# rezasalatin/PINN_depthEstimation

Hardware: AMD Instinct MI355X
Metric: collocation-point residuals/sec (fwd+PDE-grad+Adam) (higher is better)
Workload: dtype f32; 1 GPU; BASELINE configs[1]: 3->8x64 tanh->4 MLP, Navier_Stokes residual, 1048576 synthetic (t,x,y) points per GPU, full-batch Adam step; points_per_gpu=1048576, global_points=1048576, params=29636, parallelism=dp1, engine=0, allreduce_bytes=0

## Files before the change

pinn_depthestimation_amd/csrc/fused_kernel.h:

```cpp
#pragma once
#include <string.h>
#include <type_traits>
#include "common.h"
#include "residuals.h"

namespace pinn {

typedef float f4 __attribute__((ext_vector_type(4)));

constexpr int FUSED_WAVES = 4;
constexpr int FUSED_W16_WAVES = 3;
constexpr int FUSED_FLUSH_ROWS = 4;
constexpr int FUSED_THREADS = FUSED_WAVES * 64;
constexpr int TB_FLOATS = 256;
constexpr int TB_PER_WAVE = 8;
constexpr int MAX_SUMS = 12;
constexpr int MSE_SUM0 = 4;

struct FusedParams {
  int d_in, d_out, L, act;
  int dir_col[PINN_MAX_DIRS];
  int64_t N, n_tiles;
  const float* X;
  const float* Wp;
  const float* WTp;
  const float* Bp;
  float* scratch;
  int64_t scratch_per_wave;
  float* Y; float* dY;
  int loss_kind;
  int residual_id;
  int out_col[PINN_MAX_ROLES];
  int q_of[PINN_MAX_DIRS];
  float thr, anchor; int xcol;
  const float* scale;
  int n_cols;
  int mse_col[PINN_MAX_ROLES];
  const float* T;
  int64_t n_split;
  const float* mse_scale;
  float* wg_sums;
  float* wg_grads;
  int acc_lds;
  int PW, PB;
  int lds_acc_floats;
  int batch_T;
  int io1;
  uint32_t drop_seed, drop_thresh;
  float drop_scale, drop_keep;
  const float* gY;
  const float* gdY;
};

inline void set_residual_roles(FusedParams& P, const Net& n, const pinn_residual_spec& spec) {
  P.residual_id = spec.residual_id;
  for (int j = 0; j < PINN_MAX_ROLES; ++j) P.out_col[j] = spec.out_col[j];
  for (int d = 0; d < PINN_MAX_DIRS; ++d) P.q_of[d] = 1 + spec.dir_of[d];
  P.thr = spec.param[0]; P.anchor = spec.param[1];
  P.xcol = n.dir_col[spec.dir_of[0]];
}
inline void set_loss(FusedParams& P, const Net& n, const LossReq& rq) {
  P.n_split = rq.n_split;
  P.loss_kind = rq.kind == 0 ? 1 : (rq.kind == 1 ? 2 : 3);
  if (P.loss_kind & 1) { P.scale = rq.scale; set_residual_roles(P, n, rq.spec); }
  else for (int j = 0; j < PINN_MAX_ROLES; ++j) P.out_col[j] = -1;
  if (P.loss_kind & 2) {
    P.n_cols = rq.n_cols; P.T = rq.T; P.mse_scale = rq.mse_scale;
    for (int j = 0; j < PINN_MAX_ROLES; ++j) P.mse_col[j] = j < rq.n_cols ? rq.out_col[j] : -1;
  }
}

__device__ __forceinline__ f4 mfma4(float a, float b, f4 c) {
  return __builtin_amdgcn_mfma_f32_16x16x4f32(a, b, c, 0, 0, 0);
}

template <int WP> __device__ __forceinline__ int w_off_p(int l) { return l == 0 ? 0 : WP * 16 + (l - 1) * WP * WP; }
template <int WP> __device__ __forceinline__ int b_off_p(int l) { return l * WP; }

template <int NT_IN, int NT_OUT>
__device__ __forceinline__ void load_w(const float* __restrict__ Wl, f4 (&w)[NT_OUT][NT_IN], int m, int kq) {
  constexpr int LDW = 16 * NT_IN;
#pragma unroll
  for (int MT = 0; MT < NT_OUT; ++MT)
#pragma unroll
    for (int kt = 0; kt < NT_IN; ++kt)
      w[MT][kt] = *reinterpret_cast<const f4*>(Wl + (16 * MT + m) * LDW + 16 * kt + 4 * kq);
}

template <int NT_IN, int NT_OUT, int K1, int KR = 4>
__device__ __forceinline__ void gemm_chain(const f4 (&w)[NT_OUT][NT_IN], const f4 (&bin)[K1][NT_IN],
                                           f4 (&acc)[K1][NT_OUT]) {
#pragma unroll
  for (int MT = 0; MT < NT_OUT; ++MT)
#pragma unroll
    for (int kt = 0; kt < NT_IN; ++kt)
#pragma unroll
      for (int r = 0; r < KR; ++r)
#pragma unroll
        for (int c = 0; c < K1; ++c) acc[c][MT] = mfma4(w[MT][kt][r], bin[c][kt][r], acc[c][MT]);
}


template <int NT_IN>
__device__ __forceinline__ void load_wblk(const float* __restrict__ Wl, int MT, f4 (&w)[NT_IN], int m, int kq) {
#pragma unroll
  for (int kt = 0; kt < NT_IN; ++kt)
    w[kt] = *reinterpret_cast<const f4*>(Wl + (16 * MT + m) * (16 * NT_IN) + 16 * kt + 4 * kq);
}

struct NoMid { __device__ __forceinline__ void operator()() const {} };
template <int NT_IN, int NT_OUT, int K1, class Mid = NoMid>
__device__ __forceinline__ void gemm_stream(const float* __restrict__ Wl, const float* __restrict__ Wnext,
                                            f4 (&wa)[NT_IN], const f4 (&bin)[K1][NT_IN], f4 (&acc)[K1][NT_OUT],
                                            int m, int kq, const Mid& mid = Mid()) {
  constexpr int MID_BLOCK = NT_OUT >= 3 ? 1 : 0;
#pragma unroll
  for (int MT = 0; MT < NT_OUT; ++MT) {
    f4 wb[NT_IN];
    if (MT + 1 < NT_OUT) load_wblk<NT_IN>(Wl, MT + 1, wb, m, kq);
    else load_wblk<NT_IN>(Wnext, 0, wb, m, kq);
    if (MT == MID_BLOCK) mid();
#pragma unroll
    for (int kt = 0; kt < NT_IN; ++kt)
#pragma unroll
      for (int r = 0; r < 4; ++r)
#pragma unroll
        for (int c = 0; c < K1; ++c) acc[c][MT] = mfma4(wa[kt][r], bin[c][kt][r], acc[c][MT]);
    __builtin_amdgcn_sched_barrier(0);
#pragma unroll
    for (int kt = 0; kt < NT_IN; ++kt) wa[kt] = wb[kt];
  }
}

template <int NT, int K1>
__device__ __forceinline__ void zero_tiles(f4 (&v)[K1][NT]) {
#pragma unroll
  for (int c = 0; c < K1; ++c)
#pragma unroll
    for (int MT = 0; MT < NT; ++MT) v[c][MT] = f4{0.f, 0.f, 0.f, 0.f};
}

template <int NT, int K1>
__device__ __forceinline__ void init_bias(const float* __restrict__ b, f4 (&acc)[K1][NT], int q) {
#pragma unroll
  for (int MT = 0; MT < NT; ++MT) {
    acc[0][MT] = *reinterpret_cast<const f4*>(b + 16 * MT + 4 * q);
#pragma unroll
    for (int c = 1; c < K1; ++c) acc[c][MT] = f4{0.f, 0.f, 0.f, 0.f};
  }
}

template <int ACT, int NT, int K1>
__device__ __forceinline__ void activate(f4 (&acc)[K1][NT]) {
#pragma unroll
  for (int MT = 0; MT < NT; ++MT)
#pragma unroll
    for (int r = 0; r < 4; ++r) {
      const float z = acc[0][MT][r];
      float a, s;
      if constexpr (ACT == PINN_ACT_TANH) { a = tanh_f32(z); s = fmaf(-a, a, 1.f); }
      else { a = z > 0.f ? z : 0.01f * z; s = z > 0.f ? 1.f : 0.01f; }
      acc[0][MT][r] = a;
#pragma unroll
      for (int c = 1; c < K1; ++c) acc[c][MT][r] *= s;
    }
}

template <int ACT, int NT, int K1>
__device__ __forceinline__ void activate_adjoint(f4 (&G)[K1][NT], const f4 (&A)[K1][NT]) {
#pragma unroll
  for (int MT = 0; MT < NT; ++MT)
#pragma unroll
    for (int r = 0; r < 4; ++r) {
      const float a = A[0][MT][r];
      if constexpr (ACT == PINN_ACT_TANH) {
        const float s = fmaf(-a, a, 1.f);
        float cross = 0.f;
#pragma unroll
        for (int c = 1; c < K1; ++c) {
          cross = fmaf(G[c][MT][r], A[c][MT][r], cross);
          G[c][MT][r] *= s;
        }
        G[0][MT][r] = fmaf(-2.f * a, cross, s * G[0][MT][r]);
      } else {
        const float s = a > 0.f ? 1.f : 0.01f;
#pragma unroll
        for (int c = 0; c < K1; ++c) G[c][MT][r] *= s;
      }
    }
}


struct DropLane {
  uint32_t h0, hi, thresh;
  float scale, keep_p;
  __device__ __forceinline__ void init(uint32_t seed, uint32_t thr, float sc, float kp, int64_t point) {
    h0 = dropout_fmix(seed ^ ((uint32_t)point * 0x9E3779B1u));
    hi = (uint32_t)((uint64_t)point >> 32);
    thresh = thr; scale = sc; keep_p = kp;
  }
  __device__ __forceinline__ float mask(int layer, int unit) const {
    const uint32_t x = h0 ^ (((uint32_t)layer * 0x01000193u + (uint32_t)unit) * 0x9E3779B1u + hi);
    return dropout_fmix(x) >= thresh ? scale : 0.f;
  }
};

template <int NT>
__device__ __forceinline__ void load_bias(const float* __restrict__ b, f4 (&bias)[NT], int q) {
#pragma unroll
  for (int MT = 0; MT < NT; ++MT) bias[MT] = *reinterpret_cast<const f4*>(b + 16 * MT + 4 * q);
}
template <int ACT, int NT, int K1, bool DROP = false>
__device__ __forceinline__ void activate_to(const f4 (&acc)[K1][NT], const f4 (&bias)[NT], f4 (&a)[K1][NT],
                                            const DropLane* dl = nullptr, int layer = 0, int q = 0) {
  if constexpr (ACT == PINN_ACT_TANH && !DROP) {
#pragma unroll
    for (int MT = 0; MT < NT; ++MT)
#pragma unroll
      for (int h = 0; h < 4; h += 2) {
        const f2 z = f2{acc[0][MT][h], acc[0][MT][h + 1]} + f2{bias[MT][h], bias[MT][h + 1]};
        const f2 av = tanh_f32x2(z);
        const f2 s = __builtin_elementwise_fma(-av, av, f2{1.f, 1.f});
        a[0][MT][h] = av[0]; a[0][MT][h + 1] = av[1];
#pragma unroll
        for (int c = 1; c < K1; ++c) {
          const f2 t = f2{acc[c][MT][h], acc[c][MT][h + 1]} * s;
          a[c][MT][h] = t[0]; a[c][MT][h + 1] = t[1];
        }
      }
    return;
  }
#pragma unroll
  for (int MT = 0; MT < NT; ++MT)
#pragma unroll
    for (int r = 0; r < 4; ++r) {
      const float z = acc[0][MT][r] + bias[MT][r];
      float av, s;
      if constexpr (ACT == PINN_ACT_TANH) { av = tanh_f32(z); s = fmaf(-av, av, 1.f); }
      else { av = z > 0.f ? z : 0.01f * z; s = z > 0.f ? 1.f : 0.01f; }
      if constexpr (DROP) {
        const float m = dl->mask(layer, 16 * MT + 4 * q + r);
        av *= m; s *= m;
      }
      a[0][MT][r] = av;
#pragma unroll
      for (int c = 1; c < K1; ++c) a[c][MT][r] = acc[c][MT][r] * s;
    }
}
template <int ACT, int NT, int K1, bool DROP = false>
__device__ __forceinline__ void activate_adjoint_to(const f4 (&G)[K1][NT], const f4 (&A)[K1][NT], f4 (&Z)[K1][NT],
                                                    const DropLane* dl = nullptr, int layer = 0, int q = 0) {
#pragma unroll
  for (int MT = 0; MT < NT; ++MT)
#pragma unroll
    for (int r = 0; r < 4; ++r) {
      float a = A[0][MT][r];
      if constexpr (DROP) a *= dl->keep_p;
      if constexpr (ACT == PINN_ACT_TANH) {
        float s = fmaf(-a, a, 1.f);
        if constexpr (DROP) s *= dl->mask(layer, 16 * MT + 4 * q + r);
        float cross = 0.f;
#pragma unroll
        for (int c = 1; c < K1; ++c) {
          cross = fmaf(G[c][MT][r], A[c][MT][r], cross);
          Z[c][MT][r] = G[c][MT][r] * s;
        }
        Z[0][MT][r] = fmaf(-2.f * a, cross, s * G[0][MT][r]);
      } else {
        const float s = a > 0.f ? 1.f : 0.01f;
#pragma unroll
        for (int c = 0; c < K1; ++c) Z[c][MT][r] = G[c][MT][r] * s;
      }
    }
}

template <int NT, int K1>
__device__ __forceinline__ void activate_sin_to(const f4 (&acc)[K1][NT], const f4 (&bias)[NT], f4 (&a)[K1][NT],
                                                const float* __restrict__ W0, const float* __restrict__ xrow, int d_in, int q) {
#pragma unroll
  for (int MT = 0; MT < NT; ++MT)
#pragma unroll
    for (int r = 0; r < 4; ++r) {
      float sn, cs;
      sincos_f64arg(sin_layer_z(W0 + (16 * MT + 4 * q + r) * 16, bias[MT][r], xrow, d_in), sn, cs);
      a[0][MT][r] = sn;
#pragma unroll
      for (int c = 1; c < K1; ++c) a[c][MT][r] = acc[c][MT][r] * cs;
    }
}
template <int NT, int K1, int KRI>
__device__ __forceinline__ void sin_adjoint_to(const float* __restrict__ W0, const float* __restrict__ B0, const f4 (&in)[K1][1],
                                               const f4 (&G)[K1][NT], f4 (&Z)[K1][NT], int p, int q,
                                               const float* __restrict__ xrow, int d_in) {
  f4 w0[NT][1];
  load_w<1, NT>(W0, w0, p, q);
  f4 bias[NT];
  load_bias<NT>(B0, bias, q);
  f4 cz[NT], sz[NT], cross[NT];
#pragma unroll
  for (int MT = 0; MT < NT; ++MT) {
    cross[MT] = f4{0.f, 0.f, 0.f, 0.f};
#pragma unroll
    for (int r = 0; r < 4; ++r) {
      float sn, cs;
      sincos_f64arg(sin_layer_z(W0 + (16 * MT + 4 * q + r) * 16, bias[MT][r], xrow, d_in), sn, cs);
      sz[MT][r] = sn; cz[MT][r] = cs;
    }
  }
#pragma unroll
  for (int c = 1; c < K1; ++c) {
    f4 bv[1][1], zd[1][NT];
    bv[0][0] = in[c][0];
    zero_tiles<NT, 1>(zd);
    gemm_chain<1, NT, 1, KRI>(w0, bv, zd);
#pragma unroll
    for (int MT = 0; MT < NT; ++MT)
#pragma unroll
      for (int r = 0; r < 4; ++r) {
        cross[MT][r] = fmaf(G[c][MT][r], zd[0][MT][r], cross[MT][r]);
        Z[c][MT][r] = G[c][MT][r] * cz[MT][r];
      }
  }
#pragma unroll
  for (int MT = 0; MT < NT; ++MT)
#pragma unroll
    for (int r = 0; r < 4; ++r) Z[0][MT][r] = fmaf(-sz[MT][r], cross[MT][r], cz[MT][r] * G[0][MT][r]);
}

template <int NT, int K1>
__device__ __forceinline__ void spill(float* __restrict__ slot, const f4 (&v)[K1][NT], int lane) {
#pragma unroll
  for (int c = 0; c < K1; ++c)
#pragma unroll
    for (int MT = 0; MT < NT; ++MT) *reinterpret_cast<f4*>(slot + (c * NT + MT) * 256 + lane * 4) = v[c][MT];
}
template <int NT, int K1>
__device__ __forceinline__ void unspill(const float* __restrict__ slot, f4 (&v)[K1][NT], int lane) {
#pragma unroll
  for (int c = 0; c < K1; ++c)
#pragma unroll
    for (int MT = 0; MT < NT; ++MT) v[c][MT] = *reinterpret_cast<const f4*>(slot + (c * NT + MT) * 256 + lane * 4);
}

__device__ __forceinline__ void transpose_write(float* __restrict__ tb, f4 v, int p, int q) {
  *reinterpret_cast<f4*>(tb + p * 16 + 4 * (q ^ (p & 3))) = v;
}
template <bool CONSECUTIVE = false>
__device__ __forceinline__ f4 transpose_read(const float* __restrict__ tb, int p, int q) {
  f4 o;
#pragma unroll
  for (int s = 0; s < 4; ++s) {
    const int pt = CONSECUTIVE ? 4 * q + s : 4 * s + q;
    o[s] = tb[pt * 16 + 4 * ((p >> 2) ^ (pt & 3)) + (p & 3)];
  }
  return o;
}

__device__ __forceinline__ void transpose_write2(float* __restrict__ tb, f4 v, int p, int q) {
  float* d = tb + (4 * q) * 16 + 4 * (((p >> 2) + 2 * q) & 3) + (p & 3);
#pragma unroll
  for (int r = 0; r < 4; ++r) d[r * 16] = v[r];
}
__device__ __forceinline__ f4 transpose_read2(const float* __restrict__ tb, int p, int q) {
  return *reinterpret_cast<const f4*>(tb + p * 16 + 4 * ((q + 2 * (p >> 2)) & 3));
}

__device__ __forceinline__ float add_xor16(float t) {
  const auto r = __builtin_amdgcn_permlane16_swap(__float_as_uint(t), __float_as_uint(t), false, false);
  return __uint_as_float(r[0]) + __uint_as_float(r[1]);
}
__device__ __forceinline__ float add_xor32(float t) {
  const auto r = __builtin_amdgcn_permlane32_swap(__float_as_uint(t), __float_as_uint(t), false, false);
  return __uint_as_float(r[0]) + __uint_as_float(r[1]);
}

constexpr int MAX_LOCKS = 128;

template <bool LDSACC>
struct GradSink {
  static constexpr bool LDS = LDSACC;
  float* acc;
  int* locks;
  __device__ __forceinline__ void lock(int l, int lane) const {
    if (lane == 0) {
      int expected = 0;
      while (!__hip_atomic_compare_exchange_strong(locks + l, &expected, 1, __ATOMIC_ACQUIRE, __ATOMIC_RELAXED,
                                                   __HIP_MEMORY_SCOPE_WORKGROUP)) {
        expected = 0;
        __builtin_amdgcn_s_sleep(1);
      }
    }
    __builtin_amdgcn_fence(__ATOMIC_ACQUIRE, "workgroup");
    __builtin_amdgcn_wave_barrier();
  }
  __device__ __forceinline__ void unlock(int l, int lane) const {
    __builtin_amdgcn_wave_barrier();
    __builtin_amdgcn_fence(__ATOMIC_RELEASE, "workgroup");
    if (lane == 0) __hip_atomic_store(locks + l, 0, __ATOMIC_RELEASE, __HIP_MEMORY_SCOPE_WORKGROUP);
  }
  __device__ __forceinline__ void add1(int idx, float v) const { acc[idx] += v; }
};

template <int MT_N, int NT_N, int K1, bool UNIT_A = false, class Sink>
__device__ __forceinline__ void weight_grad(const Sink& sink, int layer, int woff, int boff, const f4 (&Z)[K1][MT_N],
                                            const f4 (&A)[K1][NT_N], float* __restrict__ tb, int lane,
                                            const int* __restrict__ dir_col = nullptr) {
  static_assert(!UNIT_A || NT_N == 1, "unit tangents: the layer-0 input block");
  const int p = lane & 15, q = lane >> 4;
  f4 dw[MT_N][NT_N];
  float bs[MT_N], bcur[MT_N];
#pragma unroll
  for (int MT = 0; MT < MT_N; ++MT)
#pragma unroll
    for (int NT = 0; NT < NT_N; ++NT) dw[MT][NT] = f4{0.f, 0.f, 0.f, 0.f};
  f4 early[Sink::LDS ? 1 : MT_N][Sink::LDS ? 1 : NT_N];
  if constexpr (!Sink::LDS) {
    sink.lock(layer, lane);
#pragma unroll
    for (int MT = 0; MT < MT_N; ++MT)
#pragma unroll
      for (int NT = 0; NT < NT_N; ++NT)
        early[MT][NT] = *reinterpret_cast<const f4*>(sink.acc + woff + ((MT * NT_N + NT) * 64 + lane) * 4);
  }
  f4 zt[2][MT_N], at[2][NT_N];
  auto stage = [&](int c, f4 (&z)[MT_N], f4 (&a)[NT_N]) {
#pragma unroll
    for (int MT = 0; MT < MT_N; ++MT) transpose_write2(tb + MT * TB_FLOATS, Z[c][MT], p, q);
    const bool unit = UNIT_A && c > 0;
    if (!unit) {
#pragma unroll
      for (int NT = 0; NT < NT_N; ++NT) transpose_write2(tb + (4 + NT) * TB_FLOATS, A[c][NT], p, q);
    }
#pragma unroll
    for (int MT = 0; MT < MT_N; ++MT) z[MT] = transpose_read2(tb + MT * TB_FLOATS, p, q);
    if (!unit) {
#pragma unroll
      for (int NT = 0; NT < NT_N; ++NT) a[NT] = transpose_read2(tb + (4 + NT) * TB_FLOATS, p, q);
    } else {
      const float e = (p == dir_col[c - 1]) ? 1.f : 0.f;
      a[0] = f4{e, e, e, e};
    }
  };
  stage(0, zt[0], at[0]);
#pragma unroll
  for (int c = 0; c < K1; ++c) {
    __builtin_amdgcn_sched_barrier(0);
    if (c + 1 < K1) stage(c + 1, zt[(c + 1) & 1], at[(c + 1) & 1]);
    __builtin_amdgcn_sched_barrier(0);
    if (c == 0) {
#pragma unroll
      for (int MT = 0; MT < MT_N; ++MT) bs[MT] = (zt[0][MT][0] + zt[0][MT][1]) + (zt[0][MT][2] + zt[0][MT][3]);
    }
#pragma unroll
    for (int s = 0; s < 4; ++s)
#pragma unroll
      for (int MT = 0; MT < MT_N; ++MT)
#pragma unroll
        for (int NT = 0; NT < NT_N; ++NT) dw[MT][NT] = mfma4(zt[c & 1][MT][s], at[c & 1][NT][s], dw[MT][NT]);
  }
#pragma unroll
  for (int MT = 0; MT < MT_N; ++MT) {
    bs[MT] = add_xor32(add_xor16(bs[MT]));
  }
  if constexpr (!Sink::LDS) {
#pragma unroll
    for (int MT = 0; MT < MT_N; ++MT)
#pragma unroll
      for (int NT = 0; NT < NT_N; ++NT)
        *reinterpret_cast<f4*>(sink.acc + woff + ((MT * NT_N + NT) * 64 + lane) * 4) = early[MT][NT] + dw[MT][NT];
  } else {
    sink.lock(layer, lane);
    constexpr int FR = FUSED_FLUSH_ROWS < MT_N ? FUSED_FLUSH_ROWS : MT_N;
#pragma unroll
    for (int M0 = 0; M0 < MT_N; M0 += FR) {
      f4 cur[FR][NT_N];
#pragma unroll
      for (int MT = M0; MT < M0 + FR && MT < MT_N; ++MT)
#pragma unroll
        for (int NT = 0; NT < NT_N; ++NT)
          cur[MT - M0][NT] = *reinterpret_cast<const f4*>(sink.acc + woff + ((MT * NT_N + NT) * 64 + lane) * 4);
      if (M0 == 0) {
#pragma unroll
        for (int MT = 0; MT < MT_N; ++MT) bcur[MT] = sink.acc[boff + 16 * MT + p];
      }
      __builtin_amdgcn_sched_barrier(0);
      __builtin_amdgcn_sched_barrier(0);
#pragma unroll
      for (int MT = M0; MT < M0 + FR && MT < MT_N; ++MT)
#pragma unroll
        for (int NT = 0; NT < NT_N; ++NT)
          *reinterpret_cast<f4*>(sink.acc + woff + ((MT * NT_N + NT) * 64 + lane) * 4) = cur[MT - M0][NT] + dw[MT][NT];
    }
  }
  if (q == 0) {
#pragma unroll
    for (int MT = 0; MT < MT_N; ++MT) {
      if constexpr (Sink::LDS) sink.acc[boff + 16 * MT + p] = bcur[MT] + bs[MT];
      else sink.add1(boff + 16 * MT + p, bs[MT]);
    }
  }
  sink.unlock(layer, lane);
}

__device__ __forceinline__ float pick4(f4 v, int i) {
  return i == 0 ? v[0] : (i == 1 ? v[1] : (i == 2 ? v[2] : v[3]));
}
__device__ __forceinline__ float gather_out(f4 tile, int o, int p) {
  return __shfl(pick4(tile, o & 3), p + 16 * (o >> 2), 64);
}
__device__ __forceinline__ f4 select4(bool take, f4 a, f4 b) { return take ? a : b; }
template <int K1>
__device__ __forceinline__ f4 pick_q(const f4 (&out)[K1][1], int qi) {
  f4 v = out[0][0];
#pragma unroll
  for (int c = 1; c < K1; ++c) v = select4(qi == c, out[c][0], v);
  return v;
}

template <int K1>
struct ScatterMap {
  int role_of[4];
  int cinv[K1];
};

template <int K1, int NC, int NR, bool ACCUM = false>
__device__ __forceinline__ void scatter_adjoint(float* __restrict__ tb, const float (&g)[NC][NR],
                                                const ScatterMap<K1>& sm, f4 (&G)[K1][1], bool valid, int p, int q) {
  if (q == 0) {
#pragma unroll
    for (int c = 0; c < NC; ++c)
#pragma unroll
      for (int r = 0; r < NR; ++r) tb[(c * NR + r) * 16 + p] = g[c][r];
  }
  __builtin_amdgcn_wave_barrier();
#pragma unroll
  for (int ce = 0; ce < K1; ++ce)
#pragma unroll
    for (int r2 = 0; r2 < 4; ++r2) {
      const int ci = sm.cinv[ce], ro = sm.role_of[r2];
      const bool ok = valid && ci >= 0 && ci < NC && ro >= 0;
      const float val = tb[ok ? (ci * NR + ro) * 16 + p : p];
      G[ce][0][r2] = (ACCUM ? G[ce][0][r2] : 0.f) + (ok ? val : 0.f);
    }
  __builtin_amdgcn_wave_barrier();
}

template <class RES, int K1, bool GRAD>
__device__ __forceinline__ void residual_tile(const FusedParams& P, const f4 (&out)[K1][1], f4 (&G)[K1][1],
                                              float (&sums)[MAX_SUMS], const ScatterMap<K1>& sm,
                                              float* __restrict__ tb, bool valid, bool masked, int p, int q,
                                              bool primary = true) {
  constexpr int NR = RES::NR, ND = RES::ND, NT = RES::NT;
  float v[1 + ND][NR], g[1 + ND][NR], sq[NT], sc[NT];
#pragma unroll
  for (int c = 0; c <= ND; ++c) {
    const f4 tile = (c == 0) ? out[0][0] : pick_q<K1>(out, P.q_of[c - 1]);
#pragma unroll
    for (int r = 0; r < NR; ++r) v[c][r] = gather_out(tile, P.out_col[r], p);
  }
#pragma unroll
  for (int t = 0; t < NT; ++t) sc[t] = GRAD ? P.scale[t] : 0.f;
  if constexpr (std::is_same<RES, ResContinuity>::value)
    RES::template eval<GRAD>(v, sc, g, sq, P.residual_id == PINN_RES_CONTINUITY_ONLY, masked, P.anchor);
  else
    RES::template eval<GRAD>(v, sc, g, sq);
  if (valid && q == 0 && primary) {
#pragma unroll
    for (int t = 0; t < NT; ++t) sums[t] += sq[t];
  }
  if constexpr (GRAD) scatter_adjoint<K1, 1 + ND, NR>(tb, g, sm, G, valid, p, q);
}

template <int K1>
__device__ __forceinline__ void build_scatter_maps(const FusedParams& P, int q, ScatterMap<K1>& sm, ScatterMap<K1>& sm_mse) {
#pragma unroll
  for (int r2 = 0; r2 < 4; ++r2) {
    int ro = -1, rm = -1;
    for (int r = PINN_MAX_ROLES - 1; r >= 0; --r) {
      ro = (P.out_col[r] == 4 * q + r2) ? r : ro;
      rm = (r < P.n_cols && P.mse_col[r] == 4 * q + r2) ? r : rm;
    }
    sm.role_of[r2] = ro;
    sm_mse.role_of[r2] = rm;
  }
  sm.cinv[0] = 0; sm_mse.cinv[0] = 0;
#pragma unroll
  for (int ce = 1; ce < K1; ++ce) {
    int ci = -1;
    for (int d = PINN_MAX_DIRS - 1; d >= 0; --d) ci = (P.q_of[d] == ce) ? 1 + d : ci;
    sm.cinv[ce] = ci;
    sm_mse.cinv[ce] = -1;
  }
}

constexpr int EPI_GENERIC = 0, EPI_NS = 1, EPI_PE = 2, EPI_CONT = 3, EPI_ADJ = 4, EPI_FIELD = 5, EPI_PEC = 6, EPI_FIELD_PEC = 7,
              EPI_COEF = 8, EPI_WEIGHTED = 9;
constexpr int COEF_SUM = 3;

template <int K1>
__device__ __forceinline__ void load_adjoint(const FusedParams& P, f4 (&G)[K1][1], int64_t pt, bool valid, int q) {
#pragma unroll
  for (int r = 0; r < 4; ++r) {
    const int o = 4 * q + r;
    const bool ok = valid && o < P.d_out;
    G[0][0][r] = (ok && P.gY != nullptr) ? P.gY[pt * P.d_out + o] : 0.f;
#pragma unroll
    for (int c = 1; c < K1; ++c)
      G[c][0][r] = (ok && P.gdY != nullptr) ? P.gdY[((int64_t)(c - 1) * P.N + pt) * P.d_out + o] : 0.f;
  }
}

template <class RES, int K1>
// ... 307 lines not shown
```

pinn_depthestimation_amd/csrc/fused_tile_body.inc:

```
  constexpr bool IO1 = KRO > 0;
  constexpr int KRI = IO1 ? 1 : 4;
  constexpr int KRL = IO1 ? KRO : 4;
  extern __shared__ __attribute__((aligned(16))) float smem[];
  constexpr int NTH = WP / 16;
  constexpr bool SIN0 = ACT == PINN_ACT_SIN_TANH;
  constexpr int ACT_H = SIN0 ? PINN_ACT_TANH : ACT;
  const int lane = threadIdx.x & 63, wave = threadIdx.x >> 6;
  const int p = lane & 15, q = lane >> 4;
  float* lacc = smem;
  int* locks = reinterpret_cast<int*>(smem + P.lds_acc_floats);
  float* tb = smem + P.lds_acc_floats + MAX_LOCKS + wave * (TB_PER_WAVE * TB_FLOATS);
  float* lsum = smem + P.lds_acc_floats + MAX_LOCKS + FUSED_WAVES * TB_PER_WAVE * TB_FLOATS;
  const int PP = P.PW + P.PB;
  GradSink<LDSACC> sink;
  sink.acc = LDSACC ? lacc : P.wg_grads + (int64_t)blockIdx.x * PP;
  sink.locks = locks;
  if (GRAD) {
    if (LDSACC) {
      for (int i = threadIdx.x; i < PP; i += FUSED_THREADS) lacc[i] = 0.f;
    }
    if (threadIdx.x < MAX_LOCKS) locks[threadIdx.x] = 0;
    __syncthreads();
  }
  float sums[MAX_SUMS];
#pragma unroll
  for (int j = 0; j < MAX_SUMS; ++j) sums[j] = 0.f;

  ScatterMap<K1> sm, sm_mse;
  build_scatter_maps<K1>(P, q, sm, sm_mse);
  const int nw = gridDim.x * FUSED_WAVES;
  const int gw = EPI == EPI_ADJ ? wave * (int)gridDim.x + (int)blockIdx.x : (int)blockIdx.x * FUSED_WAVES + wave;
  float* __restrict__ scr = P.scratch + (int64_t)gw * P.scratch_per_wave;
  const float* __restrict__ Wp_ = P.Wp;
  const float* __restrict__ WTp_ = P.WTp;
  const float* __restrict__ Bp_ = P.Bp;
  constexpr int SLOT = K1 * NTH * 256;
  const int L = P.L;

#ifdef PINN_DIAG
  unsigned long long diag[12] = {0, 0, 0, 0, 0, 0, 0, 0, 0, 0, 0, 0}, tprev = __builtin_amdgcn_s_memtime();
#endif
  auto load_x = [&](int64_t t, f4& x) {
    int64_t pc = t * 16 + p;
    pc = pc < P.N ? pc : P.N - 1;
#pragma unroll
    for (int r = 0; r < 4; ++r) {
      const int f = IO1 ? (r == 0 ? q : 16) : 4 * q + r;
      x[r] = (f < P.d_in) ? P.X[pc * P.d_in + f] : 0.f;
    }
  };
  f4 xnext;
  load_x(gw < P.n_tiles ? gw : 0, xnext);
  for (int64_t tile = gw; tile < P.n_tiles; tile += nw) {
    PINN_STAMP(11);
    const int64_t pt = tile * 16 + p;
    const bool valid = pt < P.N;
    const int64_t ptc = valid ? pt : P.N - 1;
    DropLane dl;
    if constexpr (DROP) dl.init(P.drop_seed, P.drop_thresh, P.drop_scale, P.drop_keep, pt);
    const f4 xcur = {finite_input(xnext[0]), finite_input(xnext[1]), finite_input(xnext[2]), finite_input(xnext[3])};
    load_x(tile + nw < P.n_tiles ? tile + nw : tile, xnext);
    auto input_jet = [&](f4 (&b)[K1][1]) {
#pragma unroll
      for (int r = 0; r < 4; ++r) {
        const int f = 4 * q + r;
        b[0][0][r] = xcur[r];
#pragma unroll
        for (int c = 1; c < K1; ++c) b[c][0][r] = (f == P.dir_col[c - 1]) ? 1.f : 0.f;
      }
    };
    f4 b0[K1][1];
    input_jet(b0);
    f4 a[K1][NTH];
    f4 ws[NTH];
    {
      f4 w0[NTH][1];
      load_w<1, NTH>(Wp_, w0, p, q);
      load_wblk<NTH>(Wp_ + w_off_p<WP>(L > 1 ? 1 : L), 0, ws, p, q);
      f4 bias[NTH];
      load_bias<NTH>(Bp_ + b_off_p<WP>(0), bias, q);
      f4 acc0[K1][NTH];
      zero_tiles<NTH, K1>(acc0);
      gemm_chain<1, NTH, K1, KRI>(w0, b0, acc0);
      PINN_STAMP(0);
      if constexpr (SIN0) activate_sin_to<NTH, K1>(acc0, bias, a, Wp_, P.X + ptc * P.d_in, P.d_in, q);
      else activate_to<ACT, NTH, K1, DROP>(acc0, bias, a, &dl, 0, q);
    }
    PINN_STAMP(1);
    for (int l = 1; l < L; ++l) {
      f4 bias[NTH];
      load_bias<NTH>(Bp_ + b_off_p<WP>(l), bias, q);
      f4 nx[K1][NTH];
      zero_tiles<NTH, K1>(nx);
      auto sp = [&]() { if (GRAD) spill<NTH, K1>(scr + (l - 1) * SLOT, a, lane); };
      gemm_stream<NTH, NTH, K1>(Wp_ + w_off_p<WP>(l), Wp_ + w_off_p<WP>(l + 1), ws, a, nx, p, q, sp);
      PINN_STAMP(0);
      activate_to<ACT_H, NTH, K1, DROP>(nx, bias, a, &dl, l, q);
      PINN_STAMP(1);
    }
    f4 G[K1][1];
    f4 out[K1][1];
    if constexpr (EPI == EPI_ADJ) {
      load_adjoint<K1>(P, G, pt, valid, q);
      load_wblk<NTH>(WTp_ + w_off_p<WP>(L > 1 ? L - 1 : 0), 0, ws, p, q);
    } else {
      f4 bias_o[1];
      load_bias<1>(Bp_ + b_off_p<WP>(L), bias_o, q);
      zero_tiles<1, K1>(out);
      gemm_stream<NTH, 1, K1>(Wp_ + w_off_p<WP>(L), WTp_ + w_off_p<WP>(L > 1 ? L - 1 : 0), ws, a, out, p, q);
      out[0][0] += bias_o[0];
    }
    f4 wtl[NTH][1];
    f4 ai[K1][NTH];
    if constexpr (GRAD) load_w<1, NTH>(WTp_ + w_off_p<WP>(L), wtl, p, q);

    if constexpr (EPI == EPI_FIELD) field_epilogue<K1>(P, out, pt, ptc, valid, p, q);
    else if constexpr (EPI == EPI_FIELD_PEC) field_tile<ResPhysicsEquationCorrected, K1>(P, out, pt, valid, false, p, q);
    else if constexpr (EPI == EPI_COEF) coef_epilogue<K1, GRAD>(P, out, G, sums, sm, tb, valid, p, q);
    else if constexpr (EPI == EPI_WEIGHTED) weighted_epilogue<K1, GRAD>(P, out, G, sums, sm, tb, pt, ptc, valid, p, q);
    else if constexpr (EPI != EPI_ADJ) loss_epilogue<K1, GRAD, (WP < 64 || EPI == EPI_PEC), EPI>(P, out, G, sums, sm, sm_mse, tb, pt, ptc, valid, p, q);

    PINN_STAMP(2);
    if constexpr (GRAD) {
      weight_grad<1, NTH, K1>(sink, L, w_off_p<WP>(L), P.PW + b_off_p<WP>(L), G, a, tb, lane);
      f4 z[K1][NTH];
      {
        f4 g[K1][NTH];
        zero_tiles<NTH, K1>(g);
        gemm_chain<1, NTH, K1, KRL>(wtl, G, g);
        if constexpr (SIN0) {
          if (L == 1) { f4 b1[K1][1]; input_jet(b1); sin_adjoint_to<NTH, K1, KRI>(Wp_, Bp_ + b_off_p<WP>(0), b1, g, z, p, q, P.X + ptc * P.d_in, P.d_in); }
          else activate_adjoint_to<ACT_H, NTH, K1, DROP>(g, a, z, &dl, L - 1, q);
        } else activate_adjoint_to<ACT, NTH, K1, DROP>(g, a, z, &dl, L - 1, q);
      }
      for (int l = L - 1; l >= 1; --l) {
        PINN_STAMP(3);
        f4 g2[K1][NTH];
        zero_tiles<NTH, K1>(g2);
        auto ld = [&]() { unspill<NTH, K1>(scr + (l - 1) * SLOT, ai, lane); };
        gemm_stream<NTH, NTH, K1>(WTp_ + w_off_p<WP>(l), WTp_ + w_off_p<WP>(l >= 2 ? l - 1 : 1), ws, z, g2, p, q, ld);
        PINN_STAMP(6);
        weight_grad<NTH, NTH, K1>(sink, l, w_off_p<WP>(l), P.PW + b_off_p<WP>(l), z, ai, tb, lane);
        PINN_STAMP(5);
        if constexpr (SIN0) {
          if (l == 1) { f4 b1[K1][1]; input_jet(b1); sin_adjoint_to<NTH, K1, KRI>(Wp_, Bp_ + b_off_p<WP>(0), b1, g2, z, p, q, P.X + ptc * P.d_in, P.d_in); }
          else activate_adjoint_to<ACT_H, NTH, K1, DROP>(g2, ai, z, &dl, l - 1, q);
        } else activate_adjoint_to<ACT, NTH, K1, DROP>(g2, ai, z, &dl, l - 1, q);
        PINN_STAMP(4);
      }
      {
        f4 b1[K1][1];
        input_jet(b1);
        weight_grad<NTH, 1, K1, LDSACC>(sink, 0, 0, P.PW + b_off_p<WP>(0), z, b1, tb, lane, P.dir_col);
      }
    }
    PINN_STAMP(7);
  }
#ifdef PINN_DIAG
  if (blockIdx.x == 0 && threadIdx.x == 0 && GRAD) {
    unsigned long long tot = 0;
    for (int i = 0; i < 12; ++i) tot += diag[i];
    printf("DIAG cycles/wave: fwd_gemm %llu fwd_act+spill %llu out+residual %llu | unspill_wait %llu adjoint %llu wgrad(transp+mfma+flush) %llu bwd_gemm %llu first/last-layer %llu loop-top %llu | total %llu\n",
           diag[0], diag[1], diag[2], diag[3], diag[4], diag[5], diag[6], diag[7], diag[11], tot);
  }
#endif

  if constexpr (EPI == EPI_FIELD || EPI == EPI_FIELD_PEC) return;
#pragma unroll
  for (int j = 0; j < MAX_SUMS; ++j) {
    float v = sums[j];
#pragma unroll
    for (int off = 32; off > 0; off >>= 1) v += __shfl_down(v, off, 64);
    if (lane == 0) lsum[wave * MAX_SUMS + j] = v;
  }
  __syncthreads();
  if (threadIdx.x < MAX_SUMS) {
    float v = 0.f;
#pragma unroll
    for (int w = 0; w < FUSED_WAVES; ++w) v += lsum[w * MAX_SUMS + threadIdx.x];
    P.wg_sums[(int64_t)blockIdx.x * MAX_SUMS + threadIdx.x] = v;
  }
  if (GRAD && LDSACC) {
    float* dst = P.wg_grads + (int64_t)blockIdx.x * PP;
    for (int i = threadIdx.x; i < PP; i += FUSED_THREADS) dst[i] = lacc[i];
  }
```

pinn_depthestimation_amd/csrc/pinn_fused_plain.hip:

```cpp
#include "fused_kernel.h"

namespace pinn {

constexpr int plain4_occ(int WP) { return WP == 64 ? 2 : 4; }

template <int WP, int ACT>
__global__ __launch_bounds__(FUSED_THREADS, plain4_occ(WP)) void k_fused_plain4(const FusedParams P) {
  constexpr int NTH = WP / 16, C = 4;
  const int lane = threadIdx.x & 63, wave = threadIdx.x >> 6;
  const int p = lane & 15, q = lane >> 4;
  const int64_t gw = (int64_t)blockIdx.x * FUSED_WAVES + wave, nw = (int64_t)gridDim.x * FUSED_WAVES;
  const float* __restrict__ Wp_ = P.Wp;
  const float* __restrict__ Bp_ = P.Bp;
  const int L = P.L;
  const int64_t n_groups = (P.n_tiles + C - 1) / C;
  for (int64_t g = gw; g < n_groups; g += nw) {
    int64_t pt[C];
    f4 b0[C][1];
#pragma unroll
    for (int c = 0; c < C; ++c) {
      pt[c] = (g * C + c) * 16 + p;
      const int64_t pc = pt[c] < P.N ? pt[c] : P.N - 1;
#pragma unroll
      for (int r = 0; r < 4; ++r) {
        const int f = 4 * q + r;
        b0[c][0][r] = f < P.d_in ? finite_input(P.X[pc * P.d_in + f]) : 0.f;
      }
    }
    f4 a[C][NTH];
    f4 ws[NTH];
    {
      f4 w0[NTH][1];
      load_w<1, NTH>(Wp_, w0, p, q);
      load_wblk<NTH>(Wp_ + w_off_p<WP>(L > 1 ? 1 : L), 0, ws, p, q);
      f4 bias[NTH];
      load_bias<NTH>(Bp_ + b_off_p<WP>(0), bias, q);
      f4 acc0[C][NTH];
      zero_tiles<NTH, C>(acc0);
      gemm_chain<1, NTH, C>(w0, b0, acc0);
#pragma unroll
      for (int c = 0; c < C; ++c)
#pragma unroll
        for (int MT = 0; MT < NTH; ++MT)
#pragma unroll
          for (int r = 0; r < 4; ++r) {
            const float z = acc0[c][MT][r] + bias[MT][r];
            if constexpr (ACT == PINN_ACT_SIN_TANH) {
              const int64_t pc = pt[c] < P.N ? pt[c] : P.N - 1;
              float sn, cs;
              sincos_f64arg(sin_layer_z(Wp_ + (16 * MT + 4 * q + r) * 16, bias[MT][r], P.X + pc * P.d_in, P.d_in), sn, cs);
              a[c][MT][r] = sn;
            }
            else a[c][MT][r] = ACT == PINN_ACT_TANH ? tanh_f32(z) : (z > 0.f ? z : 0.01f * z);
          }
    }
    for (int l = 1; l < L; ++l) {
      f4 bias[NTH];
      load_bias<NTH>(Bp_ + b_off_p<WP>(l), bias, q);
      f4 nx[C][NTH];
      zero_tiles<NTH, C>(nx);
      gemm_stream<NTH, NTH, C>(Wp_ + w_off_p<WP>(l), Wp_ + w_off_p<WP>(l + 1), ws, a, nx, p, q);
#pragma unroll
      for (int c = 0; c < C; ++c)
#pragma unroll
        for (int MT = 0; MT < NTH; ++MT)
#pragma unroll
          for (int r = 0; r < 4; ++r) {
            const float z = nx[c][MT][r] + bias[MT][r];
            a[c][MT][r] = (ACT == PINN_ACT_TANH || ACT == PINN_ACT_SIN_TANH) ? tanh_f32(z) : (z > 0.f ? z : 0.01f * z);
          }
    }
    f4 out[C][1];
    {
      f4 bias_o[1];
      load_bias<1>(Bp_ + b_off_p<WP>(L), bias_o, q);
      zero_tiles<1, C>(out);
      gemm_stream<NTH, 1, C>(Wp_ + w_off_p<WP>(L), Wp_ + w_off_p<WP>(L > 1 ? 1 : L), ws, a, out, p, q);
#pragma unroll
      for (int c = 0; c < C; ++c) out[c][0] += bias_o[0];
    }
#pragma unroll
    for (int c = 0; c < C; ++c) {
      if (pt[c] < P.N) {
#pragma unroll
        for (int r = 0; r < 4; ++r) {
          const int o = 4 * q + r;
          if (o < P.d_out) P.Y[pt[c] * P.d_out + o] = out[c][0][r];
        }
      }
    }
  }
}

template <int WP>
static int launch_plain(const FusedParams& P, int64_t n_tiles, int cus, hipStream_t s) {
  const int64_t want = ((n_tiles + 3) / 4 + FUSED_WAVES - 1) / FUSED_WAVES, cap = (int64_t)plain4_occ(WP) * cus;
  const int grid = (int)(want < cap ? want : cap);
  if (P.act == PINN_ACT_TANH) hipLaunchKernelGGL((k_fused_plain4<WP, PINN_ACT_TANH>), dim3(grid), dim3(FUSED_THREADS), 0, s, P);
  else if (P.act == PINN_ACT_SIN_TANH) hipLaunchKernelGGL((k_fused_plain4<WP, PINN_ACT_SIN_TANH>), dim3(grid), dim3(FUSED_THREADS), 0, s, P);
  else if (P.act != PINN_ACT_LEAKY_RELU) { set_error("fused plain-forward kernel: no instance for activation %d", P.act); return PINN_ERR_UNSUPPORTED; }
  else hipLaunchKernelGGL((k_fused_plain4<WP, PINN_ACT_LEAKY_RELU>), dim3(grid), dim3(FUSED_THREADS), 0, s, P);
  return check_launch("fused plain-forward kernel (four tiles per wave)");
}

int64_t fused_plain_min_tiles(int WP, int cus) { return (int64_t)4 * FUSED_WAVES * plain4_occ(WP) * cus; }

int launch_fused_plain(int WP, const FusedParams& P, int cus, hipStream_t s) {
  return WP == 16 ? launch_plain<16>(P, P.n_tiles, cus, s) : WP == 32 ? launch_plain<32>(P, P.n_tiles, cus, s)
                                                                        : launch_plain<64>(P, P.n_tiles, cus, s);
}

}
```

pinn_depthestimation_amd/csrc/pinn_fused_sin.inc:

```
#include <type_traits>
#include "fused_kernel.h"

namespace pinn {

constexpr int WP_ = FUSED_WP;

template <class K>
static int sgo(K kern, const FusedParams& P, int grid, size_t lds, hipStream_t s, const char* what) {
  if (int rc = ensure_dynamic_lds(reinterpret_cast<const void*>(kern), lds)) return rc;
  hipLaunchKernelGGL(kern, dim3(grid), dim3(FUSED_THREADS), lds, s, P);
  return check_launch(what);
}

template <int K1>
static int launch_sin_k(bool grad, const FusedParams& P, int grid, size_t lds, hipStream_t s, const char* what) {
  if (!grad) return sgo(k_fused<WP_, K1, false, false, PINN_ACT_SIN_TANH, EPI_GENERIC>, P, grid, lds, s, what);
  return P.acc_lds ? sgo(k_fused<WP_, K1, true, true, PINN_ACT_SIN_TANH, EPI_GENERIC>, P, grid, lds, s, what)
                   : sgo(k_fused<WP_, K1, true, false, PINN_ACT_SIN_TANH, EPI_GENERIC>, P, grid, lds, s, what);
}

template <>
int launch_fused_sin<WP_>(int K1, bool grad, const FusedParams& P, int grid, size_t lds, hipStream_t s) {
  const char* what = WP_ == 16 ? "fused kernel (WP=16, sine first layer)" : WP_ == 32 ? "fused kernel (WP=32, sine first layer)"
                                                                                       : "fused kernel (WP=64, sine first layer)";
  if (P.act != PINN_ACT_SIN_TANH) { set_error("fused engine: the sine instances serve activation 2 only (got %d)", P.act); return PINN_ERR_UNSUPPORTED; }
  if (K1 == 4) return launch_sin_k<4>(grad, P, grid, lds, s, what);
  if (K1 == 3) return launch_sin_k<3>(grad, P, grid, lds, s, what);
  if (K1 == 1) return launch_sin_k<1>(grad, P, grid, lds, s, what);
  set_error("fused engine: no sine-first-layer kernel for k = %d", K1 - 1);
  return PINN_ERR_UNSUPPORTED;
}

}
```

Baseline: 169.3 million residual-points/s.

## Interleave weight loads, bias loads, spills and LDS transposes evenly among MFMAs

Replaces the block-wise issue of next-block weight loads, bias loads and activation spills in gemm_stream with a compile-time pacing scheme. It spreads these memory ops across the MFMA sequence at a fixed gap, separated by sched_barriers. weight_grad similarly splits the LDS transpose staging for the next derivative channel into half-writes and reads threaded between the outer-product MFMAs. The aim is to hide load and LDS latency behind matrix work for WP>=64. It also moves one sine kernel instance into its own translation unit to split compilation, at the cost of extra schedule constraints and template complexity.

After: 172.8 million residual-points/s (median of 6 runs). 1.02x the previous value.

```diff
diff --git a/pinn_depthestimation_amd/csrc/fused_kernel.h b/pinn_depthestimation_amd/csrc/fused_kernel.h
--- a/pinn_depthestimation_amd/csrc/fused_kernel.h
+++ b/pinn_depthestimation_amd/csrc/fused_kernel.h
@@ -109,27 +109,78 @@
 }
 
 struct NoMid { __device__ __forceinline__ void operator()() const {} };
-template <int NT_IN, int NT_OUT, int K1, class Mid = NoMid>
+
+template <int I, int N, class F>
+__device__ __forceinline__ void const_for(F&& f) {
+  if constexpr (I < N) {
+    f(std::integral_constant<int, I>{});
+    const_for<I + 1, N>(f);
+  }
+}
+struct NoOps {
+  static constexpr int COUNT = 0;
+  template <int J> __device__ __forceinline__ void op() const {}
+};
+template <int NT, int K1, bool ON = true>
+struct SpillOps {
+  static constexpr int COUNT = ON ? K1 * NT : 0;
+  float* __restrict__ slot;
+  const f4 (&v)[K1][NT];
+  int lane;
+  template <int J> __device__ __forceinline__ void op() const { *reinterpret_cast<f4*>(slot + J * 256 + lane * 4) = v[J / NT][J % NT]; }
+};
+template <int NT, int K1>
+struct UnspillOps {
+  static constexpr int COUNT = K1 * NT;
+  const float* __restrict__ slot;
+  f4 (&v)[K1][NT];
+  int lane;
+  template <int J> __device__ __forceinline__ void op() const { v[J / NT][J % NT] = *reinterpret_cast<const f4*>(slot + J * 256 + lane * 4); }
+};
+template <int NT>
+struct BiasOps {
+  static constexpr int COUNT = NT;
+  const float* __restrict__ b;
+  f4 (&bias)[NT];
+  int q;
+  template <int J> __device__ __forceinline__ void op() const { bias[J] = *reinterpret_cast<const f4*>(b + 16 * J + 4 * q); }
+};
+constexpr int PACE_GAP = 2, PACE_OFF = 1 << 20, PACE_MIN_WP = 64;
+template <int NT_IN, int NT_OUT, int K1, class Mid = NoOps, class Head = NoOps, int GAP = PACE_GAP>
 __device__ __forceinline__ void gemm_stream(const float* __restrict__ Wl, const float* __restrict__ Wnext,
                                             f4 (&wa)[NT_IN], const f4 (&bin)[K1][NT_IN], f4 (&acc)[K1][NT_OUT],
-                                            int m, int kq, const Mid& mid = Mid()) {
+                                            int m, int kq, const Mid& mid = Mid(), const Head& head = Head()) {
   constexpr int MID_BLOCK = NT_OUT >= 3 ? 1 : 0;
-#pragma unroll
-  for (int MT = 0; MT < NT_OUT; ++MT) {
+  constexpr int NM = NT_IN * 4 * K1;
+  constexpr int NSLOT = (NM + GAP - 1) / GAP;
+  const_for<0, NT_OUT>([&](auto mt_) {
+    constexpr int MT = decltype(mt_)::value;
+    constexpr int NHEAD = MT == 0 ? Head::COUNT : 0, NMID = MT == MID_BLOCK ? Mid::COUNT : 0;
+    constexpr int NOPS = NT_IN + NHEAD + NMID;
     f4 wb[NT_IN];
-    if (MT + 1 < NT_OUT) load_wblk<NT_IN>(Wl, MT + 1, wb, m, kq);
-    else load_wblk<NT_IN>(Wnext, 0, wb, m, kq);
-    if (MT == MID_BLOCK) mid();
-#pragma unroll
-    for (int kt = 0; kt < NT_IN; ++kt)
-#pragma unroll
-      for (int r = 0; r < 4; ++r)
-#pragma unroll
-        for (int c = 0; c < K1; ++c) acc[c][MT] = mfma4(wa[kt][r], bin[c][kt][r], acc[c][MT]);
+    const float* __restrict__ wsrc = (MT + 1 < NT_OUT ? Wl + (16 * (MT + 1) + m) * (16 * NT_IN) : Wnext + m * (16 * NT_IN)) + 4 * kq;
+    const_for<0, NM>([&](auto i_) {
+      constexpr int i = decltype(i_)::value;
+      if constexpr (i % GAP == 0) {
+        constexpr int S = i / GAP;
+        constexpr int K_LO = NOPS <= NSLOT ? (S < NOPS ? S : NOPS) : (S * NOPS + NSLOT - 1) / NSLOT;
+        constexpr int K_HI = NOPS <= NSLOT ? (S + 1 < NOPS ? S + 1 : NOPS) : ((S + 1) * NOPS + NSLOT - 1) / NSLOT;
+        if constexpr (K_HI > K_LO && i > 0) __builtin_amdgcn_sched_barrier(0);
+        const_for<K_LO, K_HI>([&](auto k_) {
+          constexpr int k = decltype(k_)::value;
+          if constexpr (k < NT_IN) wb[k] = *reinterpret_cast<const f4*>(wsrc + 16 * k);
+          else if constexpr (k < NT_IN + NHEAD) head.template op<k - NT_IN>();
+          else mid.template op<k - NT_IN - NHEAD>();
+        });
+        if constexpr (K_HI > K_LO && NSLOT > 1) __builtin_amdgcn_sched_barrier(0);
+      }
+      constexpr int kt = i / (4 * K1), r = (i / K1) % 4, c = i % K1;
+      acc[c][MT] = mfma4(wa[kt][r], bin[c][kt][r], acc[c][MT]);
+    });
     __builtin_amdgcn_sched_barrier(0);
 #pragma unroll
     for (int kt = 0; kt < NT_IN; ++kt) wa[kt] = wb[kt];
-  }
+  });
 }
 
 template <int NT, int K1>
@@ -327,21 +378,6 @@
     for (int r = 0; r < 4; ++r) Z[0][MT][r] = fmaf(-sz[MT][r], cross[MT][r], cz[MT][r] * G[0][MT][r]);
 }
 
-template <int NT, int K1>
-__device__ __forceinline__ void spill(float* __restrict__ slot, const f4 (&v)[K1][NT], int lane) {
-#pragma unroll
-  for (int c = 0; c < K1; ++c)
-#pragma unroll
-    for (int MT = 0; MT < NT; ++MT) *reinterpret_cast<f4*>(slot + (c * NT + MT) * 256 + lane * 4) = v[c][MT];
-}
-template <int NT, int K1>
-__device__ __forceinline__ void unspill(const float* __restrict__ slot, f4 (&v)[K1][NT], int lane) {
-#pragma unroll
-  for (int c = 0; c < K1; ++c)
-#pragma unroll
-    for (int MT = 0; MT < NT; ++MT) v[c][MT] = *reinterpret_cast<const f4*>(slot + (c * NT + MT) * 256 + lane * 4);
-}
-
 __device__ __forceinline__ void transpose_write(float* __restrict__ tb, f4 v, int p, int q) {
   *reinterpret_cast<f4*>(tb + p * 16 + 4 * (q ^ (p & 3))) = v;
 }
@@ -356,10 +392,15 @@
   return o;
 }
 
+template <int H>
+__device__ __forceinline__ void transpose_write2_half(float* __restrict__ tb, f4 v, int p, int q) {
+  float* d = tb + (4 * q) * 16 + 4 * (((p >> 2) + 2 * q) & 3) + (p & 3);
+  d[(2 * H) * 16] = v[2 * H];
+  d[(2 * H + 1) * 16] = v[2 * H + 1];
+}
 __device__ __forceinline__ void transpose_write2(float* __restrict__ tb, f4 v, int p, int q) {
-  float* d = tb + (4 * q) * 16 + 4 * (((p >> 2) + 2 * q) & 3) + (p & 3);
-#pragma unroll
-  for (int r = 0; r < 4; ++r) d[r * 16] = v[r];
+  transpose_write2_half<0>(tb, v, p, q);
+  transpose_write2_half<1>(tb, v, p, q);
 }
 __device__ __forceinline__ f4 transpose_read2(const float* __restrict__ tb, int p, int q) {
   return *reinterpret_cast<const f4*>(tb + p * 16 + 4 * ((q + 2 * (p >> 2)) & 3));
@@ -401,7 +442,7 @@
   __device__ __forceinline__ void add1(int idx, float v) const { acc[idx] += v; }
 };
 
-template <int MT_N, int NT_N, int K1, bool UNIT_A = false, class Sink>
+template <int MT_N, int NT_N, int K1, bool UNIT_A = false, bool PACED = true, class Sink>
 __device__ __forceinline__ void weight_grad(const Sink& sink, int layer, int woff, int boff, const f4 (&Z)[K1][MT_N],
                                             const f4 (&A)[K1][NT_N], float* __restrict__ tb, int lane,
                                             const int* __restrict__ dir_col = nullptr) {
@@ -423,41 +464,48 @@
         early[MT][NT] = *reinterpret_cast<const f4*>(sink.acc + woff + ((MT * NT_N + NT) * 64 + lane) * 4);
   }
   f4 zt[2][MT_N], at[2][NT_N];
-  auto stage = [&](int c, f4 (&z)[MT_N], f4 (&a)[NT_N]) {
-#pragma unroll
-    for (int MT = 0; MT < MT_N; ++MT) transpose_write2(tb + MT * TB_FLOATS, Z[c][MT], p, q);
-    const bool unit = UNIT_A && c > 0;
-    if (!unit) {
-#pragma unroll
-      for (int NT = 0; NT < NT_N; ++NT) transpose_write2(tb + (4 + NT) * TB_FLOATS, A[c][NT], p, q);
-    }
-#pragma unroll
-    for (int MT = 0; MT < MT_N; ++MT) z[MT] = transpose_read2(tb + MT * TB_FLOATS, p, q);
-    if (!unit) {
-#pragma unroll
-      for (int NT = 0; NT < NT_N; ++NT) a[NT] = transpose_read2(tb + (4 + NT) * TB_FLOATS, p, q);
+  auto stage_op = [&](auto c_, auto k_, f4 (&z)[MT_N], f4 (&a)[NT_N]) {
+    constexpr int c = decltype(c_)::value, k = decltype(k_)::value;
+    constexpr int NB = MT_N + ((UNIT_A && c > 0) ? 0 : NT_N);
+    if constexpr (k < 2 * NB) {
+      constexpr int B = k / 2;
+      if constexpr (B < MT_N) transpose_write2_half<k % 2>(tb + B * TB_FLOATS, Z[c][B], p, q);
+      else transpose_write2_half<k % 2>(tb + (4 + B - MT_N) * TB_FLOATS, A[c][B - MT_N], p, q);
     } else {
-      const float e = (p == dir_col[c - 1]) ? 1.f : 0.f;
-      a[0] = f4{e, e, e, e};
+      constexpr int B = k - 2 * NB;
+      if constexpr (B < MT_N) z[B] = transpose_read2(tb + B * TB_FLOATS, p, q);
+      else a[B - MT_N] = transpose_read2(tb + (4 + B - MT_N) * TB_FLOATS, p, q);
     }
   };
-  stage(0, zt[0], at[0]);
-#pragma unroll
-  for (int c = 0; c < K1; ++c) {
+  auto unit_operand = [&](int c, f4 (&a)[NT_N]) {
+    const float e = (p == dir_col[c - 1]) ? 1.f : 0.f;
+    a[0] = f4{e, e, e, e};
+  };
+  const_for<0, 3 * (MT_N + NT_N)>([&](auto k_) { stage_op(std::integral_constant<int, 0>{}, k_, zt[0], at[0]); });
+  constexpr int NM = 4 * MT_N * NT_N;
+  constexpr int SPAN = PACED ? NM - (NM >= 8 ? NM / 8 : 1) : 1;
+  const_for<0, K1>([&](auto c_) {
+    constexpr int c = decltype(c_)::value;
+    constexpr int NOPS = c + 1 < K1 ? 3 * (MT_N + ((UNIT_A && c + 1 > 0) ? 0 : NT_N)) : 0;
     __builtin_amdgcn_sched_barrier(0);
-    if (c + 1 < K1) stage(c + 1, zt[(c + 1) & 1], at[(c + 1) & 1]);
+    if constexpr (UNIT_A && c + 1 < K1) unit_operand(c + 1, at[(c + 1) & 1]);
+    if constexpr (c == 0) {
+#pragma unroll
+      for (int MT = 0; MT < MT_N; ++MT) bs[MT] = (zt[0][MT][0] + zt[0][MT][1]) + (zt[0][MT][2] + zt[0][MT][3]);
+    }
     __builtin_amdgcn_sched_barrier(0);
-    if (c == 0) {
-#pragma unroll
-      for (int MT = 0; MT < MT_N; ++MT) bs[MT] = (zt[0][MT][0] + zt[0][MT][1]) + (zt[0][MT][2] + zt[0][MT][3]);
-    }
-#pragma unroll
-    for (int s = 0; s < 4; ++s)
-#pragma unroll
-      for (int MT = 0; MT < MT_N; ++MT)
-#pragma unroll
-        for (int NT = 0; NT < NT_N; ++NT) dw[MT][NT] = mfma4(zt[c & 1][MT][s], at[c & 1][NT][s], dw[MT][NT]);
-  }
+    const_for<0, NM>([&](auto i_) {
+      constexpr int i = decltype(i_)::value;
+      if constexpr (i < SPAN && NOPS > 0) {
+        constexpr int K_LO = (i * NOPS + SPAN - 1) / SPAN, K_HI = ((i + 1) * NOPS + SPAN - 1) / SPAN;
+        if constexpr (K_HI > K_LO && i > 0) __builtin_amdgcn_sched_barrier(0);
+        const_for<K_LO, K_HI>([&](auto k_) { stage_op(std::integral_constant<int, c + 1>{}, k_, zt[(c + 1) & 1], at[(c + 1) & 1]); });
+        if constexpr (K_HI > K_LO && PACED) __builtin_amdgcn_sched_barrier(0);
+      }
+      constexpr int s = i / (MT_N * NT_N), MT = (i / NT_N) % MT_N, NT = i % NT_N;
+      dw[MT][NT] = mfma4(zt[c & 1][MT][s], at[c & 1][NT][s], dw[MT][NT]);
+    });
+  });
 #pragma unroll
   for (int MT = 0; MT < MT_N; ++MT) {
     bs[MT] = add_xor32(add_xor16(bs[MT]));
diff --git a/pinn_depthestimation_amd/csrc/fused_tile_body.inc b/pinn_depthestimation_amd/csrc/fused_tile_body.inc
--- a/pinn_depthestimation_amd/csrc/fused_tile_body.inc
+++ b/pinn_depthestimation_amd/csrc/fused_tile_body.inc
@@ -1,3 +1,5 @@
+  constexpr bool PACED = WP >= PACE_MIN_WP;
+  constexpr int GAP_FWD = PACED ? PACE_GAP : PACE_OFF;
   constexpr bool IO1 = KRO > 0;
   constexpr int KRI = IO1 ? 1 : 4;
   constexpr int KRL = IO1 ? KRO : 4;
@@ -89,11 +91,11 @@
     PINN_STAMP(1);
     for (int l = 1; l < L; ++l) {
       f4 bias[NTH];
-      load_bias<NTH>(Bp_ + b_off_p<WP>(l), bias, q);
       f4 nx[K1][NTH];
       zero_tiles<NTH, K1>(nx);
-      auto sp = [&]() { if (GRAD) spill<NTH, K1>(scr + (l - 1) * SLOT, a, lane); };
-      gemm_stream<NTH, NTH, K1>(Wp_ + w_off_p<WP>(l), Wp_ + w_off_p<WP>(l + 1), ws, a, nx, p, q, sp);
+      const SpillOps<NTH, K1, GRAD> sp{scr + (l - 1) * SLOT, a, lane};
+      const BiasOps<NTH> lb{Bp_ + b_off_p<WP>(l), bias, q};
+      gemm_stream<NTH, NTH, K1, SpillOps<NTH, K1, GRAD>, BiasOps<NTH>, GAP_FWD>(Wp_ + w_off_p<WP>(l), Wp_ + w_off_p<WP>(l + 1), ws, a, nx, p, q, sp, lb);
       PINN_STAMP(0);
       activate_to<ACT_H, NTH, K1, DROP>(nx, bias, a, &dl, l, q);
       PINN_STAMP(1);
@@ -105,9 +107,9 @@
       load_wblk<NTH>(WTp_ + w_off_p<WP>(L > 1 ? L - 1 : 0), 0, ws, p, q);
     } else {
       f4 bias_o[1];
-      load_bias<1>(Bp_ + b_off_p<WP>(L), bias_o, q);
       zero_tiles<1, K1>(out);
-      gemm_stream<NTH, 1, K1>(Wp_ + w_off_p<WP>(L), WTp_ + w_off_p<WP>(L > 1 ? L - 1 : 0), ws, a, out, p, q);
+      const BiasOps<1> lb{Bp_ + b_off_p<WP>(L), bias_o, q};
+      gemm_stream<NTH, 1, K1, NoOps, BiasOps<1>, GAP_FWD>(Wp_ + w_off_p<WP>(L), WTp_ + w_off_p<WP>(L > 1 ? L - 1 : 0), ws, a, out, p, q, NoOps(), lb);
       out[0][0] += bias_o[0];
     }
     f4 wtl[NTH][1];
@@ -122,7 +124,7 @@
 
     PINN_STAMP(2);
     if constexpr (GRAD) {
-      weight_grad<1, NTH, K1>(sink, L, w_off_p<WP>(L), P.PW + b_off_p<WP>(L), G, a, tb, lane);
+      weight_grad<1, NTH, K1, false, PACED>(sink, L, w_off_p<WP>(L), P.PW + b_off_p<WP>(L), G, a, tb, lane);
       f4 z[K1][NTH];
       {
         f4 g[K1][NTH];
@@ -137,10 +139,10 @@
         PINN_STAMP(3);
         f4 g2[K1][NTH];
         zero_tiles<NTH, K1>(g2);
-        auto ld = [&]() { unspill<NTH, K1>(scr + (l - 1) * SLOT, ai, lane); };
-        gemm_stream<NTH, NTH, K1>(WTp_ + w_off_p<WP>(l), WTp_ + w_off_p<WP>(l >= 2 ? l - 1 : 1), ws, z, g2, p, q, ld);
+        const UnspillOps<NTH, K1> ld{scr + (l - 1) * SLOT, ai, lane};
+        gemm_stream<NTH, NTH, K1, UnspillOps<NTH, K1>, NoOps, PACE_OFF>(WTp_ + w_off_p<WP>(l), WTp_ + w_off_p<WP>(l >= 2 ? l - 1 : 1), ws, z, g2, p, q, ld);
         PINN_STAMP(6);
-        weight_grad<NTH, NTH, K1>(sink, l, w_off_p<WP>(l), P.PW + b_off_p<WP>(l), z, ai, tb, lane);
+        weight_grad<NTH, NTH, K1, false, PACED>(sink, l, w_off_p<WP>(l), P.PW + b_off_p<WP>(l), z, ai, tb, lane);
         PINN_STAMP(5);
         if constexpr (SIN0) {
           if (l == 1) { f4 b1[K1][1]; input_jet(b1); sin_adjoint_to<NTH, K1, KRI>(Wp_, Bp_ + b_off_p<WP>(0), b1, g2, z, p, q, P.X + ptc * P.d_in, P.d_in); }
@@ -151,7 +153,7 @@
       {
         f4 b1[K1][1];
         input_jet(b1);
-        weight_grad<NTH, 1, K1, LDSACC>(sink, 0, 0, P.PW + b_off_p<WP>(0), z, b1, tb, lane, P.dir_col);
+        weight_grad<NTH, 1, K1, LDSACC, PACED>(sink, 0, 0, P.PW + b_off_p<WP>(0), z, b1, tb, lane, P.dir_col);
       }
     }
     PINN_STAMP(7);
diff --git a/pinn_depthestimation_amd/csrc/pinn_fused_plain.hip b/pinn_depthestimation_amd/csrc/pinn_fused_plain.hip
--- a/pinn_depthestimation_amd/csrc/pinn_fused_plain.hip
+++ b/pinn_depthestimation_amd/csrc/pinn_fused_plain.hip
@@ -59,7 +59,7 @@
       load_bias<NTH>(Bp_ + b_off_p<WP>(l), bias, q);
       f4 nx[C][NTH];
       zero_tiles<NTH, C>(nx);
-      gemm_stream<NTH, NTH, C>(Wp_ + w_off_p<WP>(l), Wp_ + w_off_p<WP>(l + 1), ws, a, nx, p, q);
+      gemm_stream<NTH, NTH, C, NoOps, NoOps, PACE_OFF>(Wp_ + w_off_p<WP>(l), Wp_ + w_off_p<WP>(l + 1), ws, a, nx, p, q);
 #pragma unroll
       for (int c = 0; c < C; ++c)
 #pragma unroll
@@ -75,7 +75,7 @@
       f4 bias_o[1];
       load_bias<1>(Bp_ + b_off_p<WP>(L), bias_o, q);
       zero_tiles<1, C>(out);
-      gemm_stream<NTH, 1, C>(Wp_ + w_off_p<WP>(L), Wp_ + w_off_p<WP>(L > 1 ? 1 : L), ws, a, out, p, q);
+      gemm_stream<NTH, 1, C, NoOps, NoOps, PACE_OFF>(Wp_ + w_off_p<WP>(L), Wp_ + w_off_p<WP>(L > 1 ? 1 : L), ws, a, out, p, q);
 #pragma unroll
       for (int c = 0; c < C; ++c) out[c][0] += bias_o[0];
     }
diff --git a/pinn_depthestimation_amd/csrc/pinn_fused_sin.inc b/pinn_depthestimation_amd/csrc/pinn_fused_sin.inc
--- a/pinn_depthestimation_amd/csrc/pinn_fused_sin.inc
+++ b/pinn_depthestimation_amd/csrc/pinn_fused_sin.inc
@@ -4,6 +4,10 @@
 namespace pinn {
 
 constexpr int WP_ = FUSED_WP;
+
+#if FUSED_WP == 64
+extern template __global__ void k_fused<64, 4, true, false, PINN_ACT_SIN_TANH, EPI_GENERIC>(const FusedParams);
+#endif
 
 template <class K>
 static int sgo(K kern, const FusedParams& P, int grid, size_t lds, hipStream_t s, const char* what) {
diff --git a/pinn_depthestimation_amd/csrc/pinn_fused_sin_w64_g4.hip b/pinn_depthestimation_amd/csrc/pinn_fused_sin_w64_g4.hip
--- /dev/null
+++ b/pinn_depthestimation_amd/csrc/pinn_fused_sin_w64_g4.hip
@@ -0,0 +1,5 @@
+#include "fused_kernel.h"
+
+namespace pinn {
+template __global__ void k_fused<64, 4, true, false, PINN_ACT_SIN_TANH, EPI_GENERIC>(const FusedParams);
+}
```
